# kit-cel/vae-equalizer

Hardware: AMD Instinct MI355X
Metric: equalized symbols/s/GPU, DP 64-QAM VAE-LE (higher is better)
Workload: dtype f32

## Files before the change

### vae_equalizer_amd/csrc/vaeq_dp_wave_kernel.h

```cpp
#pragma once
#include <hip/hip_runtime.h>
#include <stdint.h>
#include <type_traits>

#include "vaeq.h"
#include "vaeq_common.h"
#include "vaeq_launch.h"
#include "vaeq_wave.h"

#ifdef VAEQ_PHASE_STAMPS
#define VAEQ_STAMP(i) do { if (s == a.steps - 1) tst[i] = __builtin_readcyclecounter(); } while (0)
#define VAEQ_XSTAMP(i) do { if (s == a.steps - 1) tsx[i] = __builtin_readcyclecounter(); } while (0)
#else
#define VAEQ_STAMP(i) do { } while (0)
#define VAEQ_XSTAMP(i) do { } while (0)
#endif
#define VAEQ_NSTAMP 12
#ifndef VAEQ_PIPE
#define VAEQ_PIPE 1
#endif
#define VAEQ_BT_FRAMES 16
#ifndef VAEQ_WPS
#define VAEQ_WPS 2
#endif

namespace vaeq {

__device__ __forceinline__ float half_sum(float a0, float a1)
{
    const auto r = __builtin_amdgcn_permlane32_swap(__builtin_bit_cast(unsigned, a0), __builtin_bit_cast(unsigned, a1), false, false);
    return __builtin_bit_cast(float, (unsigned)r[0]) + __builtin_bit_cast(float, (unsigned)r[1]);
}

struct WaveLayout {
    int Lph, Uph;
    int X, E, U, PSv, W, H, PSh, VS, MOM, RED, XG, total;
};

__host__ __device__ inline WaveLayout wave_layout(int B, int M, int NW = 1)
{
    WaveLayout l;
    const int len = 2 * B + M - 1;
    const int lph = wave_lph(len);
    l.Lph = lph;
    l.Uph = B / 2 + 1;
    int o = 0;
    auto take = [&](int bytes) { int r = o; o += (bytes + 15) & ~15; return r; };
    l.X = take(2 * 4 * lph * 8);
    l.E = take(2 * 4 * lph * 8);
    const int ubytes = 2 * 2 * l.Uph * 8, gbytes = 2 * B * 8;
    l.U = take(ubytes > gbytes ? ubytes : gbytes);
    l.PSv = take(2 * (B + 1) * 4);
    l.W = take(2 * M * 16);
    l.H = take(2 * 2 * (M + 1) * 8);
    l.PSh = take(2 * (M + 1) * 4);
    l.VS = take(2 * M * 4);
    l.MOM = take(16 * 64 * 4);
    l.RED = take(NW > 1 ? 64 * 4 : 0);
    l.XG = take((NW - 1) * 4 * 64 * 4);
    l.total = o;
    return l;
}

struct CellCarry {
    static constexpr int fir_off(int g, int j, int Lph) { return g + (j < 4 ? j * Lph : (j - 4) * Lph + 1); }
    static constexpr int poly4(int c, int Lph) { return (c & 3) * Lph + (c >> 2); }
    static constexpr int d3_off(int b, int d, int mh, int Uph) { return (d & 1 ? Uph : 0) + (mh >> 1) - b + (d == -1 ? -1 : d == 2 ? 1 : 0); }
    static constexpr int poly2(int c, int Uph) { return (c & 1) * Uph + (c >> 1); }
    static constexpr bool fir_exact(int B, int M)
    {
        const int G = M / 4, len = 2 * B + M - 1, Lph = wave_lph(len);
        if (M % 4 != 1 || G < 2 || G % 2) return false;
        for (int g = 0; g < G; g++)
            for (int j = 0; j < 6; j++) {
                if (fir_off(g, j, Lph) != poly4(4 * g + j, Lph)) return false;
                if (4 * (B / 2 - 1) + 4 * g + j >= len) return false;
                if (g + 1 < G && j >= 4 && fir_off(g, j, Lph) != fir_off(g + 1, j - 4, Lph)) return false;
            }
        return poly4(4 * G, Lph) == fir_off(G - 1, 4, Lph) && 4 * (B / 2 - 1) + 4 * G + 2 < len;
    }
    static constexpr bool d3_exact(int B, int M)
    {
        const int mh = M / 2, NB = (mh + 1) / 2, Uph = B / 2 + 1, T = B - mh;
        if ((mh & 1) || NB < 2 || NB % 2) return false;
// ... 359 lines not shown
    char *sm = reinterpret_cast<char *>(smem4);
    const int gl = threadIdx.x, lane = NW > 1 ? (gl & 63) : gl, wv = NW > 1 ? (gl >> 6) : 0, run = blockIdx.x;
    constexpr int NT = 64 * NW, NP = 2 * NW;
    constexpr bool UNI = BT > 0 && uniform_parts(BT, M, NP);
    constexpr bool FIXL = BT > 0 || (BL > 0 && M != 13 && M != 17 && !(M == 31 && NW == 1));
    constexpr bool PIPE = VAEQ_PIPE && FIXL;
    constexpr bool WIDE = FIXL;
    constexpr bool B100 = BT == 100 && NW == 1;
    constexpr bool CARRY = B100 && M == 25 && PIPE && WIDE;
    constexpr int QAUX = B100 ? 2 : 0;
    const int B = BT ? BT : a.B;
    const int BS = BT ? BT : BL ? BL : B;
    constexpr bool ODDB = BT == 0 && BL > 0;
    const int L = 2 * B, nm = L - Mh, P2 = ODDB ? (B + 1) / 2 : B / 2;
    const float rnm = 1.0f / (float)nm;
    const WaveLayout lay = wave_layout(BS, M, NW);
    const int Lph = lay.Lph, Uph = lay.Uph;
    float2 *Xs = reinterpret_cast<float2 *>(sm + lay.X), *Es = reinterpret_cast<float2 *>(sm + lay.E);
    float2 *Us = reinterpret_cast<float2 *>(sm + lay.U), *GY = Us;
    float4 *Wt = reinterpret_cast<float4 *>(sm + lay.W);
    float2 *Ht = reinterpret_cast<float2 *>(sm + lay.H);
    float *PSv = reinterpret_cast<float *>(sm + lay.PSv);
    float *PSh = reinterpret_cast<float *>(sm + lay.PSh);
    float *VS = reinterpret_cast<float *>(sm + lay.VS);
    float *RED = reinterpret_cast<float *>(sm + lay.RED), *XG = reinterpret_cast<float *>(sm + lay.XG);

    float amp[NLEV], b2[NLEV], nlogP[NLEV];
    const float nusc = a.nu_sc[run];
#pragma unroll
    for (int i = 0; i < NLEV; i++) {
        amp[i] = a.amp[i];
        b2[i] = nusc * amp[i] * amp[i] * LOG2E;
        nlogP[i] = -logf(a.P[(size_t)run * NLEV + i]);
    }
    const float var0 = a.var[run * 2 + 0], var1 = a.var[run * 2 + 1];
    const float lrW = a.lr_W[run], lrH = a.lr_h[run];

    for (int i = gl; i < (lay.W - lay.X) / 8; i += NT) Xs[i] = make_float2(0.f, 0.f);
    for (int i = gl; i < (lay.PSh - lay.H) / 8; i += NT) Ht[i] = make_float2(0.f, 0.f);
    __syncthreads();
    const int tk = lane & 31, half = lane >> 5;
    const bool worker = tk < M, owner = worker && wv == 0;
    const int part = wv * 2 + half;
    const size_t gbase = (size_t)run * 8 * M;
    constexpr bool TP = BT == 100 && NW == 1 && M == 25;
    int oc = half, tj = tk;
    bool ownr = owner;
    if constexpr (TP) {
        oc = TapPairMap::c(lane, M);
        tj = TapPairMap::kept(lane, M);
        ownr = TapPairMap::owns(lane, M);
    }
    float *MOM = reinterpret_cast<float *>(sm + lay.MOM) + lane;
#define mWr(p) MOM[(0 + (p)) * 64]
#define mWi(p) MOM[(2 + (p)) * 64]
#define vWr(p) MOM[(4 + (p)) * 64]
#define vWi(p) MOM[(6 + (p)) * 64]
#define mHr(p) MOM[(8 + (p)) * 64]
#define mHi(p) MOM[(10 + (p)) * 64]
#define vHr(p) MOM[(12 + (p)) * 64]
#define vHi(p) MOM[(14 + (p)) * 64]
    if (ownr) {
#pragma unroll
        for (int p = 0; p < 2; p++) {
            const size_t ir = gbase + (oc * 4 + p) * M + tj, ii = gbase + (oc * 4 + 2 + p) * M + tj;
            float *wq = reinterpret_cast<float *>(&Wt[p * M + tj]);
            wq[oc * 2 + 0] = a.W[ir];
            wq[oc * 2 + 1] = a.W[ii];
            mWr(p) = a.adam_mW[ir]; mWi(p) = a.adam_mW[ii];
            vWr(p) = a.adam_vW[ir]; vWi(p) = a.adam_vW[ii];
            const size_t hr = gbase + ((oc * 2 + p) * 2 + 0) * M + tj, hi = hr + M;
            Ht[(oc * 2 + p) * MP + tj] = make_float2(a.h[hr], a.h[hi]);
            mHr(p) = a.adam_mh[hr]; mHi(p) = a.adam_mh[hi];
            vHr(p) = a.adam_vh[hr]; vHi(p) = a.adam_vh[hi];
        }
    }
    int step = a.step[run];
    __shared__ double BTW[2][VAEQ_BT_FRAMES];
    if (gl < VAEQ_BT_FRAMES && gl < a.n_frames) {
        const double t = (double)(step + gl * a.steps);
        BTW[0][gl] = pow(0.9, t);
        BTW[1][gl] = pow(0.999, t);
    }
    __syncthreads();
    double b1t = BTW[0][0], b2t = BTW[1][0];

    const int klen = a.keep_len, k0 = a.keep_off;
    const size_t No = (size_t)a.steps * klen;
    constexpr bool pairst = PAIR;
    const bool act = gl < P2;
    const int nq = (nm + 3) / 4;
    const int n0 = 2 * gl;
    const bool v1 = ODDB ? act && (n0 + 1 < B) : act;
    const float2 *Xl = Xs + gl, *El = Es + gl, *Ul = Us + gl;
    const float2 *Xa = Xs + (act ? gl : 0), *Ea = Es + (act ? gl : 0);

    const bool ldl = gl < (ODDB ? (L + 3) / 4 : L / 4);
    float4 pf[4];
    const uint32_t S4 = (uint32_t)a.S * 4u;
    auto frame_rsrc = [&](int f) { return make_rsrc(a.rx + ((size_t)run * a.n_frames + f) * 4 * (size_t)a.S, 4u * S4); };
    auto fetch = [&](const __amdgpu_buffer_rsrc_t xr, int s) {
        const uint32_t vo = ldl ? ((uint32_t)s * (uint32_t)a.stride_sym * 2u + 4u * gl) * 4u : OOB;
#pragma unroll
        for (int r = 0; r < 4; r++) pf[r] = bld128(xr, vo, (uint32_t)r * S4);
    };
#ifdef VAEQ_PHASE_STAMPS
    long long tst[VAEQ_NSTAMP], tsx[8];
#endif
    fetch(frame_rsrc(0), 0);
    for (int f = 0; f < a.n_frames; f++) {
        const __amdgpu_buffer_rsrc_t xr = frame_rsrc(f), xn = frame_rsrc(f + 1 < a.n_frames ? f + 1 : f);
        if (f && f < VAEQ_BT_FRAMES) {
            b1t = BTW[0][f];
            b2t = BTW[1][f];
// ... 111 lines not shown
                    }
                    if (df) {
                        float v0 = q[0].x, v1 = q[0].y;
                        int b0 = 0, b1 = 0;
#pragma unroll
                        for (int i = 1; i < NLEV; i++) {
                            if (q[i].x > v0) { v0 = q[i].x; b0 = i; }
                            if (q[i].y > v1) { v1 = q[i].y; b1 = i; }
                        }
                        const uint32_t ro = (uint32_t)(o * 2 + c) * (uint32_t)No;
                        if (pairst) bst16((unsigned short)(b0 | (b1 << 8)), dr, kept0 ? col : OOB, ro);
                        else { bst8((unsigned char)b0, dr, kept0 ? col : OOB, ro); bst8((unsigned char)b1, dr, kept1 ? col + 1u : OOB, ro); }
                    }
                    v2f m2 = {0.f, 0.f}, m3 = {0.f, 0.f}, kk = {0.f, 0.f}, kl = {0.f, 0.f};
#pragma unroll
                    for (int i = 0; i < NLEV; i++) {
                        const v2f d = amp[i] - m1, qd = q[i] * d, g = z[i] * LN2 + nlogP[i];
                        m2 += qd * d;
                        m3 += qd * d * d;
                        kk += qd * g;
                        kl += q[i] * g;
                    }
                    const bool inr0 = (n0 >= mh) && (n0 < B - mh) && act;
                    const bool inr1 = (n0 + 1 >= mh) && (n0 + 1 < B - mh) && act;
                    if (inr0) klsum += kl.x - __builtin_amdgcn_logf(ssum.x) * LN2;
                    if (inr1) klsum += kl.y - __builtin_amdgcn_logf(ssum.y) * LN2;
                    asm volatile("" : "+v"(m2), "+v"(m3), "+v"(kk), "+v"(klsum));
                    mv[0][o][c] = m2.x; mv[1][o][c] = m2.y;
                    mt3[0][o][c] = m3.x; mt3[1][o][c] = m3.y;
                    mkc[0][o][c] = inr0 ? kk.x : 0.f;
                    mkc[1][o][c] = inr1 ? kk.y : 0.f;
                    if (c) { muv[0].y = m1.x; muv[1].y = m1.y; } else { muv[0].x = m1.x; muv[1].x = m1.y; }
                    if (qf) {
#pragma unroll
                        for (int i = 0; i < NLEV; i++) {
                            const uint32_t ro = qrow;
                            if (pairst) bst64<QAUX>(q[i], qr, vo0, ro);
                            else { bst32<QAUX>(q[i].x, qr, vo0, ro); bst32<QAUX>(q[i].y, qr, vo1, ro); }
                            qrow += No4;
                            asm volatile("" : "+s"(qrow));
                        }
                    }
                }
                vv[o][0] = act ? mv[0][o][0] + mv[0][o][1] : 0.f;
                vv[o][1] = v1 ? mv[1][o][0] + mv[1][o][1] : 0.f;
                if (act) {
                    Us[(o * 2 + 0) * Uph + gl] = muv[0];
                    Us[(o * 2 + 1) * Uph + gl] = v1 ? muv[1] : make_float2(0.f, 0.f);
                }
            }
            VAEQ_STAMP(4);
            {
                float inc[2];
#pragma unroll
                for (int o = 0; o < 2; o++) inc[o] = wave_incl_scan_dpp(vv[o][0] + vv[o][1]);
                if constexpr (NW > 1) {
                    if (lane == 63) { RED[wv] = inc[0]; RED[NW + wv] = inc[1]; }
                    sync_lds<NW>();
#pragma unroll
                    for (int w = 0; w < NW - 1; w++)
                        if (w < wv) { inc[0] += RED[w]; inc[1] += RED[NW + w]; }
                }
#pragma unroll
                for (int o = 0; o < 2; o++) {
                    if (act) {
                        PSv[o * (BS + 1) + n0 + 1] = inc[o] - vv[o][1];
                        PSv[o * (BS + 1) + n0 + 2] = inc[o];
                    }
                    if (gl == 0) PSv[o * (BS + 1)] = 0.f;
                }
            }
            sync_lds<NW>();
            if (owner) {
                const int lo = (Mh - tk + 1) >> 1, hi_ = (nm - 1 + Mh - tk) >> 1;
                VS[half * M + tk] = PSv[half * (BS + 1) + hi_ + 1] - PSv[half * (BS + 1) + lo];
            }
            sync_lds<NW>();

            VAEQ_STAMP(5);
            float se0 = 0.f, se1 = 0.f;
            float hq0 = 0.f, hq1 = 0.f;
            if (worker) {
                const float2 h0 = Ht[(0 * 2 + half) * MP + tk], h1 = Ht[(1 * 2 + half) * MP + tk];
                hq0 = h0.x * h0.x + h0.y * h0.y;
                hq1 = h1.x * h1.x + h1.y * h1.y;
            }
            const float vsl = worker ? VS[half * M + tk] : 0.f;
            if constexpr (B100 && M == 25) {
                constexpr int T = 100 - mh, NB = (mh + 1) / 2;
                static_assert((mh & 1) == 0 && (Mh & 3) == 0 && D3Map::exact(100, M), "D3Map: mh even (a = mh stands alone, its odd tap is the pad)");
                const int l3 = lane;
                const int m3 = D3Map::m(l3, T), modd = m3 & 1, m3h = (3 * m3) >> 1;
                cacc D3[3][2];
                const int xo = D3Map::chi(l3) * 4 * Lph + (Mh >> 2) + m3h;
                const int o0 = xo + (modd ? 2 * Lph : 0), o2 = xo + (modd ? 1 : 2 * Lph);
                const int off[6] = {o0, o0 + Lph, o2, o2 + Lph, o0 + 1, o0 + Lph + 1};
                v2f x6[6];
#pragma unroll
                for (int k = 0; k < 6; k++) x6[k] = lds2(Xs + off[k]);
                {
                    const float2 *uE = Us + modd * Uph + m3h, *uO = Us + (modd ^ 1) * Uph + m3h + modd;
                    const float2 *hc = Ht + D3Map::chi(l3) * 2 * MP;
                    v2f am[2][4];
#pragma unroll
                    for (int v = 0; v < 2; v++) {
                        am[v][0] = lds2(hc + v * MP + Mh);
                        am[v][1] = lds2(uE + v * 2 * Uph); am[v][2] = lds2(uO + v * 2 * Uph); am[v][3] = lds2(uE + v * 2 * Uph + 1);
                    }
// ... 93 lines not shown
                    const float2 *h0 = Ht + (0 * 2 + v) * MP, *h1 = Ht + (1 * 2 + v) * MP;
                    const float2 *up = Us + (gl < nq ? gl : 0) + v * 2 * Uph;
                    auto step_a = [&](int aa, v2f ulo, v2f uhi, auto first) {
                        constexpr bool F = decltype(first)::value;
                        const v2f e0 = lds2(h0 + 2 * aa), o0 = lds2(h0 + 2 * aa + 1), e1 = lds2(h1 + 2 * aa), o1 = lds2(h1 + 2 * aa + 1);
                        cmacf<F>(D[0][0], e0, ulo); cmacf<F>(D[0][1], o0, ulo);
                        cmacf<F>(D[0][2], e0, uhi); cmacf<F>(D[0][3], o0, uhi);
                        cmacf<F>(D[1][0], e1, ulo); cmacf<F>(D[1][1], o1, ulo);
                        cmacf<F>(D[1][2], e1, uhi); cmacf<F>(D[1][3], o1, uhi);
                    };
                    if (NA & 1) {
                        if (v == 0) step_a(mh, lds2(up), lds2(up + Uph), std::true_type{});
                        else step_a(mh, lds2(up), lds2(up + Uph), std::false_type{});
                    } else if (v == 0) {
#pragma unroll
                        for (int chi = 0; chi < 2; chi++)
#pragma unroll
                            for (int i = 0; i < 4; i++) D[chi][i] = cacc0();
                    }
                    constexpr int ph = mh & 1;
                    auto load = [&](int b, v2f (&r)[11]) {
                        const int sl = (mh >> 1) - b;
                        r[0] = lds2(up + ph * Uph + sl);
                        r[1] = lds2(up + (ph ^ 1) * Uph + sl + ph);
                        r[2] = lds2(up + (ph ^ 1) * Uph + sl + ph - 1);
#pragma unroll
                        for (int t = 0; t < 4; t++) { r[3 + t] = lds2(h0 + 4 * b + t); r[7 + t] = lds2(h1 + 4 * b + t); }
                    };
                    auto fma = [&](int, const v2f (&r)[11], auto) {
                        cmac(D[0][0], r[3], r[0]); cmac(D[0][1], r[4], r[0]); cmac(D[0][2], r[3], r[1]); cmac(D[0][3], r[4], r[1]);
                        cmac(D[1][0], r[7], r[0]); cmac(D[1][1], r[8], r[0]); cmac(D[1][2], r[7], r[1]); cmac(D[1][3], r[8], r[1]);
                        cmac(D[0][0], r[5], r[2]); cmac(D[0][1], r[6], r[2]); cmac(D[0][2], r[5], r[0]); cmac(D[0][3], r[6], r[0]);
                        cmac(D[1][0], r[9], r[2]); cmac(D[1][1], r[10], r[2]); cmac(D[1][2], r[9], r[0]); cmac(D[1][3], r[10], r[0]);
                    };
                    pipe2<11, false, PIPE>(NB, load, fma);
                }
                VAEQ_STAMP(6);
                if (gl < nq) {
#pragma unroll
                    for (int chi = 0; chi < 2; chi++)
#pragma unroll
                        for (int i = 0; i < 4; i++) {
                            const int ce = Mh + i;
                            const float2 x = Xl[(chi * 4 + (ce & 3)) * Lph + (ce >> 2)];
                            const float2 Dv = cfin(D[chi][i]);
                            float2 e = make_float2(x.x - Dv.x, x.y - Dv.y);
                            if (4 * gl + i >= nm) e = make_float2(0.f, 0.f);
                            Es[(chi * 4 + (ce & 3)) * Lph + gl + (ce >> 2)] = e;
                            const float e2 = e.x * e.x + e.y * e.y;
                            if (chi) se1 += e2; else se0 += e2;
                        }
                }
            }
            se0 = wave_sum_dpp(se0);
            se1 = wave_sum_dpp(se1);
            klsum = wave_sum_dpp(klsum);
            if constexpr (NW > 1) {
                if (lane == 0) { RED[16 + wv] = se0; RED[16 + NW + wv] = se1; RED[16 + 2 * NW + wv] = klsum; }
                sync_lds<NW>();
                se0 = RED[16]; se1 = RED[16 + NW]; klsum = RED[16 + 2 * NW];
#pragma unroll
                for (int w = 1; w < NW; w++) { se0 += RED[16 + w]; se1 += RED[16 + NW + w]; klsum += RED[16 + 2 * NW + w]; }
            }
            const float C0 = se0 + wave_sum_dpp(hq0 * vsl), C1 = se1 + wave_sum_dpp(hq1 * vsl);
            const float gC0 = (float)nm * __builtin_amdgcn_rcpf(C0), gC1 = (float)nm * __builtin_amdgcn_rcpf(C1);
            {
                const uint32_t vo = gl == 0 ? 0u : OOB;
                if (a.loss) bst32((float)nm * LN2 * (__builtin_amdgcn_logf(C0) + __builtin_amdgcn_logf(C1)) + klsum, lr_, vo, (uint32_t)s * 4u);
                if (a.var_est) {
                    bst32(C0 * rnm, vr_, vo, (uint32_t)s * 4u);
                    bst32(C1 * rnm, vr_, vo, ((uint32_t)a.steps + (uint32_t)s) * 4u);
                }
            }
            {
                const float inc = half_incl_scan_dpp(gC0 * hq0 + gC1 * hq1);
                if (owner) PSh[half * MP + tk + 1] = inc;
                if (tk == 0) PSh[half * MP] = 0.f;
            }
            sync_lds<NW>();

            VAEQ_STAMP(7);
            step += 1;
            b1t *= 0.9;
            b2t *= 0.999;
            const float rbc1 = __builtin_amdgcn_rcpf((float)(1.0 - b1t));
            const float bc2s = __builtin_amdgcn_rcpf(__builtin_amdgcn_sqrtf((float)(1.0 - b2t)));
            const float ssW = lrW * rbc1, ssH = lrH * rbc1;
            float2 hnew[2];
            hnew[0] = hnew[1] = make_float2(0.f, 0.f);
            float ghr[2] = {0, 0}, ghi[2] = {0, 0};
            float2 hacc[2];
            {
                float2 ph_h[2] = {make_float2(0.f, 0.f), make_float2(0.f, 0.f)};
                float ph_vs[2] = {0.f, 0.f};
                if (NW == 1 && ownr) {
#pragma unroll
                    for (int v = 0; v < 2; v++) {
                        ph_h[v] = Ht[(oc * 2 + v) * MP + tj];
                        ph_vs[v] = VS[v * M + tj];
                    }
                }
                cacc ca[2][2];
                if constexpr (TP) {
                    static_assert(TapPairMap::exact(100, M) && UNI, "TapPairMap");
                    const int lt = lane;
                    constexpr int NH = TapPairMap::dh_pairs(100, M);
                    const int par = TapPairMap::par(lt, M), sl = TapPairMap::alo(lt, M) >> 1, ma = TapPairMap::part_h(lt, M) * NH;
                    const int ceA = par + Mh, ceB = par + Mh + 2;
                    const float2 *ec = Es + TapPairMap::c(lt, M) * 4 * Lph + ma;
                    const float2 *uA = Us + (mh >> 1) - sl + ma, *uB = uA + Uph;
                    const float2 *uC = TapPairMap::tap(lt, M, 1) < M ? uB - 1 : uA;
                    VAEQ_XSTAMP(0);
                    tap_pair_sum<NH, 1>(ca, ec + (ceA & 3) * Lph + (ceA >> 2), ec + (ceB & 3) * Lph + (ceB >> 2), uA, uB, 2 * Uph, uC);
                } else {
                    const int tkc = worker ? tk : 0, par = tkc & 1, aa = tkc >> 1;
                    const int T = (nm - par + 1) >> 1, Th = ((T + 2 * NP - 1) / (2 * NP)) << 1;
                    const int ma = (part * Th) >> 1, mb = (min(T, part * Th + Th) + 1) >> 1;
                    const int ceA = par + Mh, ceB = par + Mh + 2, npA = mh - aa, npB = mh - aa + 1;
                    const float2 *eA = Es + (ceA & 3) * Lph + (ceA >> 2) + ma, *eB = Es + (ceB & 3) * Lph + (ceB >> 2) + ma;
                    const float2 *uA = Us + (npA & 1) * Uph + (npA >> 1) + ma, *uB = Us + (npB & 1) * Uph + (npB >> 1) + ma;
                    auto load1 = [&](int m, v2f *r) {
                        r[0] = lds2(eA + m); r[1] = lds2(eA + 4 * Lph + m); r[2] = lds2(uA + m); r[3] = lds2(uA + 2 * Uph + m);
                        r[4] = lds2(eB + m); r[5] = lds2(eB + 4 * Lph + m); r[6] = lds2(uB + m); r[7] = lds2(uB + 2 * Uph + m);
                    };
                    cacc cbx[2][2];
                    cacc (&cb)[2][2] = WIDE ? cbx : ca;
                    auto fma1 = [&](const v2f *r, auto first) {
                        constexpr bool F = decltype(first)::value;
                        cmacf<F>(ca[0][0], r[2], r[0]); cmacf<F>(ca[0][1], r[3], r[0]); cmacf<F>(ca[1][0], r[2], r[1]); cmacf<F>(ca[1][1], r[3], r[1]);
                        cmacf<F && WIDE>(cb[0][0], r[6], r[4]); cmacf<F && WIDE>(cb[0][1], r[7], r[4]); cmacf<F && WIDE>(cb[1][0], r[6], r[5]); cmacf<F && WIDE>(cb[1][1], r[7], r[5]);
                    };
                    auto load = [&](int i, v2f (&r)[16]) { load1(2 * i, r); load1(2 * i + 1, r + 8); };
                    auto fma = [&](int, const v2f (&r)[16], auto first) { fma1(r, first); fma1(r + 8, std::false_type{}); };
                    int n = mb - ma;
                    VAEQ_XSTAMP(0);
                    if constexpr (UNI) {
                        n = __builtin_amdgcn_readfirstlane(n);
                        pipe2<16, true, PIPE>(n >> 1, load, fma);
                    } else {
                        ca[0][0] = ca[0][1] = ca[1][0] = ca[1][1] = cbx[0][0] = cbx[0][1] = cbx[1][0] = cbx[1][1] = cacc0();
                        pipe2<16, false, PIPE>(n >> 1, load, fma);
                    }
                    if (n & 1) {
                        v2f r[8];
                        load1(n - 1, r);
                        fma1(r, std::false_type{});
                    }
                    if constexpr (WIDE) {
#pragma unroll
                        for (int i = 0; i < 2; i++)
#pragma unroll
                            for (int j = 0; j < 2; j++) { ca[i][j].a += cbx[i][j].a; ca[i][j].b += cbx[i][j].b; }
                    }
                }
                VAEQ_XSTAMP(1);
                float2 acc[2][2];
#pragma unroll
                for (int chi = 0; chi < 2; chi++)
#pragma unroll
                    for (int v = 0; v < 2; v++) acc[chi][v] = cfinc(ca[chi][v]);
                if constexpr (B100) {
#pragma unroll
                    for (int v = 0; v < 2; v++) {
                        acc[0][v].x = acc[1][v].x = half_sum(acc[0][v].x, acc[1][v].x);
                        acc[0][v].y = acc[1][v].y = half_sum(acc[0][v].y, acc[1][v].y);
                    }
                } else {
#pragma unroll
                    for (int chi = 0; chi < 2; chi++)
#pragma unroll
                        for (int v = 0; v < 2; v++) {
                            acc[chi][v].x += __shfl_xor(acc[chi][v].x, 32, 64);
                            acc[chi][v].y += __shfl_xor(acc[chi][v].y, 32, 64);
                        }
                }
                if constexpr (NW > 1) {
#pragma unroll
                    for (int v = 0; v < 2; v++) {
                        hacc[v] = half ? acc[1][v] : acc[0][v];
                        if (wv > 0) {
                            XG[((wv - 1) * 4 + 2 * v + 0) * 64 + lane] = hacc[v].x;
                            XG[((wv - 1) * 4 + 2 * v + 1) * 64 + lane] = hacc[v].y;
                        }
                    }
                }
                VAEQ_XSTAMP(2);
                if (NW == 1 && ownr) {
                    const float g = oc ? gC1 : gC0;
#pragma unroll
                    for (int v = 0; v < 2; v++) {
                        const float2 ac = half ? acc[1][v] : acc[0][v];
                        const float2 hh = ph_h[v];
                        const float vs = ph_vs[v];
                        ghr[v] = g * (-2.0f * ac.x + 2.0f * hh.x * vs);
                        ghi[v] = g * (-2.0f * ac.y + 2.0f * hh.y * vs);
                        hnew[v] = hh;
                        if (!a.no_update) {
                            adam_update_fast(hnew[v].x, mHr(v), vHr(v), ghr[v], ssH, bc2s);
                            adam_update_fast(hnew[v].y, mHi(v), vHi(v), ghi[v], ssH, bc2s);
                        }
                    }
                }
            }

            asm volatile("" : "+v"(hnew[0].x), "+v"(hnew[0].y), "+v"(hnew[1].x), "+v"(hnew[1].y), "+v"(ghr[0]), "+v"(ghr[1]), "+v"(ghi[0]),
                         "+v"(ghi[1]));
            {
                const bool last_s = s + 1 == a.steps;
                if constexpr (B100) {
                    const bool more = !(last_s && f + 1 == a.n_frames);
                    const uint32_t vo = ldl && more ? ((uint32_t)(last_s ? 0 : s + 1) * (uint32_t)a.stride_sym * 2u + 4u * gl) * 4u : OOB;
#pragma unroll
                    for (int r = 0; r < 4; r++) pf[r] = bld128(last_s ? xn : xr, vo, (uint32_t)r * S4);
                } else if (!(last_s && f + 1 == a.n_frames)) fetch(last_s ? xn : xr, last_s ? 0 : s + 1);
            }
            VAEQ_XSTAMP(3);
            VAEQ_STAMP(8);
            float2 gy[2][2];
            {
                float2 au0[2][2], au1[2][2];
                {
                    cacc cu[2][2][2];
                    pair_du<M, WIDE, CARRY>(cu, Ea, Lph, Ht, MP);
#pragma unroll
                    for (int sy = 0; sy < 2; sy++)
#pragma unroll
                        for (int v = 0; v < 2; v++) { au0[sy][v] = cfinc(cu[0][sy][v]); au1[sy][v] = cfinc(cu[1][sy][v]); }
                }
#pragma unroll
                for (int sy = 0; sy < 2; sy++) {
                    const int sx = 2 * (n0 + sy);
                    const int jlo = max(0, Mh - sx), jhi = max(jlo - 1, min(Mh, nm - 1 + Mh - sx));
#pragma unroll
                    for (int v = 0; v < 2; v++) {
                        const float ur = -2.0f * (gC0 * au0[sy][v].x + gC1 * au1[sy][v].x);
                        const float ui = -2.0f * (gC0 * au0[sy][v].y + gC1 * au1[sy][v].y);
                        const float gv = PSh[v * MP + jhi + 1] - PSh[v * MP + jlo];
                        const float iv = 1.0f / (v ? var1 : var0);
                        gy[sy][v].x = iv * (ur * mv[sy][v][0] + gv * mt3[sy][v][0] + mkc[sy][v][0]);
                        gy[sy][v].y = iv * (ui * mv[sy][v][1] + gv * mt3[sy][v][1] + mkc[sy][v][1]);
                    }
                }
            }
            VAEQ_STAMP(9);
            sync_lds<NW>();
            if constexpr (NW > 1) {
                if (owner) {
                    const float g = half ? gC1 : gC0;
#pragma unroll
                    for (int v = 0; v < 2; v++) {
                        float2 ac = hacc[v];
#pragma unroll
                        for (int w = 0; w < NW - 1; w++) {
                            ac.x += XG[(w * 4 + 2 * v + 0) * 64 + lane];
                            ac.y += XG[(w * 4 + 2 * v + 1) * 64 + lane];
                        }
                        const float2 hh = Ht[(half * 2 + v) * MP + tk];
                        const float vs = VS[v * M + tk];
                        ghr[v] = g * (-2.0f * ac.x + 2.0f * hh.x * vs);
                        ghi[v] = g * (-2.0f * ac.y + 2.0f * hh.y * vs);
                        hnew[v] = hh;
                        if (!a.no_update) {
                            adam_update_fast(hnew[v].x, mHr(v), vHr(v), ghr[v], ssH, bc2s);
                            adam_update_fast(hnew[v].y, mHi(v), vHi(v), ghi[v], ssH, bc2s);
                        }
                    }
                }
            }
            if (act) {
#pragma unroll
                for (int v = 0; v < 2; v++) {
                    GY[v * BS + n0] = gy[0][v];
                    GY[v * BS + n0 + 1] = v1 ? gy[1][v] : make_float2(0.f, 0.f);
                }
            }
            if (ownr && !a.no_update) {
                Ht[(oc * 2 + 0) * MP + tj] = hnew[0];
                Ht[(oc * 2 + 1) * MP + tj] = hnew[1];
            }
            sync_lds<NW>();

            VAEQ_STAMP(10);
            float gwr[2] = {0, 0}, gwi[2] = {0, 0};
            {
                float pw_w[2][2] = {{0.f, 0.f}, {0.f, 0.f}}, pw_m[2][2] = {{0.f, 0.f}, {0.f, 0.f}}, pw_v[2][2] = {{0.f, 0.f}, {0.f, 0.f}};
                if (ownr) {
#pragma unroll
                    for (int p = 0; p < 2; p++) {
                        const float *wq = reinterpret_cast<const float *>(&Wt[p * M + tj]) + oc * 2;
                        pw_w[p][0] = wq[0]; pw_w[p][1] = wq[1];
                        pw_m[p][0] = mWr(p); pw_m[p][1] = mWi(p);
                        pw_v[p][0] = vWr(p); pw_v[p][1] = vWi(p);
                    }
                }
                cacc ca[2][2];
                if constexpr (TP) {
                    const int lt = lane;
                    constexpr int NQ = TapPairMap::dw_pairs(100);
                    const int cA = TapPairMap::tap(lt, M, 1), cB = cA + 2, ma = TapPairMap::part_w(lt) * NQ;
                    const float2 *gA = GY + TapPairMap::c(lt, M) * BS + 2 * ma;
                    const float2 *xA = Xs + (cA & 3) * Lph + (cA >> 2) + ma, *xB = Xs + (cB & 3) * Lph + (cB >> 2) + ma;
                    cacc cr[2][2];
                    VAEQ_XSTAMP(4);
                    tap_pair_sum<NQ, 2>(cr, gA, gA + 1, xA, xB, 4 * Lph, xB - 1);
#pragma unroll
                    for (int p = 0; p < 2; p++) { ca[0][p] = cr[1][p]; ca[1][p] = cr[0][p]; }
                } else {
                    const int tkc = worker ? tk : 0;
                    const int Be = ODDB ? B + (B & 1) : B;
                    const int Bq = ((Be + 2 * NP - 1) / (2 * NP)) << 1;
                    const int ma = (part * Bq) >> 1, mb = min(Be, part * Bq + Bq) >> 1;
                    const int cA = tkc, cB = tkc + 2;
                    const float2 *xA = Xs + (cA & 3) * Lph + (cA >> 2) + ma, *xB = Xs + (cB & 3) * Lph + (cB >> 2) + ma;
                    const float2 *G0 = GY + 2 * ma, *G1 = GY + BS + 2 * ma;
                    auto load1 = [&](int m, v2f *r) {
                        r[0] = lds2(G0 + 2 * m); r[1] = lds2(G0 + 2 * m + 1); r[2] = lds2(G1 + 2 * m); r[3] = lds2(G1 + 2 * m + 1);
                        r[4] = lds2(xA + m); r[5] = lds2(xA + 4 * Lph + m); r[6] = lds2(xB + m); r[7] = lds2(xB + 4 * Lph + m);
                    };
                    cacc cbx[2][2];
                    cacc (&cb)[2][2] = WIDE ? cbx : ca;
                    auto fma1 = [&](const v2f *r, auto first) {
                        constexpr bool F = decltype(first)::value;
                        cmacf<F>(ca[0][0], r[4], r[0]); cmacf<F>(ca[0][1], r[5], r[0]); cmacf<F>(ca[1][0], r[4], r[2]); cmacf<F>(ca[1][1], r[5], r[2]);
                        cmacf<F && WIDE>(cb[0][0], r[6], r[1]); cmacf<F && WIDE>(cb[0][1], r[7], r[1]); cmacf<F && WIDE>(cb[1][0], r[6], r[3]); cmacf<F && WIDE>(cb[1][1], r[7], r[3]);
                    };
                    auto load = [&](int i, v2f (&r)[16]) { load1(2 * i, r); load1(2 * i + 1, r + 8); };
                    auto fma = [&](int, const v2f (&r)[16], auto first) { fma1(r, first); fma1(r + 8, std::false_type{}); };
                    int n = mb - ma;
                    VAEQ_XSTAMP(4);
                    if constexpr (UNI) {
                        n = __builtin_amdgcn_readfirstlane(n);
                        pipe2<16, true, PIPE>(n >> 1, load, fma);
                    } else {
                        ca[0][0] = ca[0][1] = ca[1][0] = ca[1][1] = cbx[0][0] = cbx[0][1] = cbx[1][0] = cbx[1][1] = cacc0();
                        pipe2<16, false, PIPE>(n >> 1, load, fma);
                    }
                    if (n & 1) {
                        v2f r[8];
                        load1(n - 1, r);
                        fma1(r, std::false_type{});
                    }
                    if constexpr (WIDE) {
#pragma unroll
                        for (int i = 0; i < 2; i++)
#pragma unroll
                            for (int j = 0; j < 2; j++) { ca[i][j].a += cbx[i][j].a; ca[i][j].b += cbx[i][j].b; }
                    }
                }
                VAEQ_XSTAMP(5);
                float2 acc[2][2];
#pragma unroll
                for (int o = 0; o < 2; o++)
#pragma unroll
                    for (int pp = 0; pp < 2; pp++) acc[o][pp] = cfinc(ca[o][pp]);
                if constexpr (B100) {
#pragma unroll
                    for (int p = 0; p < 2; p++) {
                        acc[0][p].x = acc[1][p].x = half_sum(acc[0][p].x, acc[1][p].x);
                        acc[0][p].y = acc[1][p].y = half_sum(acc[0][p].y, acc[1][p].y);
                    }
                } else {
#pragma unroll
                    for (int o = 0; o < 2; o++)
#pragma unroll
                        for (int p = 0; p < 2; p++) {
                            acc[o][p].x += __shfl_xor(acc[o][p].x, 32, 64);
                            acc[o][p].y += __shfl_xor(acc[o][p].y, 32, 64);
                        }
                }
                if constexpr (NW > 1) {
#pragma unroll
                    for (int p = 0; p < 2; p++) {
                        const float2 ac = half ? acc[1][p] : acc[0][p];
                        if (wv > 0) {
                            XG[((wv - 1) * 4 + 2 * p + 0) * 64 + lane] = ac.x;
                            XG[((wv - 1) * 4 + 2 * p + 1) * 64 + lane] = ac.y;
                        }
                    }
                    sync_lds<NW>();
                }
                VAEQ_XSTAMP(6);
                if (ownr) {
#pragma unroll
                    for (int p = 0; p < 2; p++) {
                        float2 ac = half ? acc[1][p] : acc[0][p];
                        if constexpr (NW > 1) {
#pragma unroll
                            for (int w = 0; w < NW - 1; w++) {
                                ac.x += XG[(w * 4 + 2 * p + 0) * 64 + lane];
                                ac.y += XG[(w * 4 + 2 * p + 1) * 64 + lane];
                            }
                        }
                        gwr[p] = ac.x;
                        gwi[p] = ac.y;
                        if (!a.no_update) {
                            float *wq = reinterpret_cast<float *>(&Wt[p * M + tj]) + oc * 2;
                            float wr = pw_w[p][0], wi = pw_w[p][1];
                            adam_update_fast(wr, pw_m[p][0], pw_v[p][0], gwr[p], ssW, bc2s);
                            adam_update_fast(wi, pw_m[p][1], pw_v[p][1], gwi[p], ssW, bc2s);
                            wq[0] = wr;
                            wq[1] = wi;
                            mWr(p) = pw_m[p][0]; mWi(p) = pw_m[p][1];
                            vWr(p) = pw_v[p][0]; vWi(p) = pw_v[p][1];
                        }
                    }
                }
            }
            if (a.dbg_gW && ownr && f == a.n_frames - 1 && s == a.steps - 1) {
#pragma unroll
                for (int p = 0; p < 2; p++) {
                    a.dbg_gW[gbase + (oc * 4 + p) * M + tj] = gwr[p];
                    a.dbg_gW[gbase + (oc * 4 + 2 + p) * M + tj] = gwi[p];
                    a.dbg_gh[gbase + ((oc * 2 + p) * 2 + 0) * M + tj] = ghr[p];
                    a.dbg_gh[gbase + ((oc * 2 + p) * 2 + 1) * M + tj] = ghi[p];
                }
            }
            sync_lds<NW>();
            VAEQ_XSTAMP(7);
            VAEQ_STAMP(11);
        }
    }
#ifdef VAEQ_PHASE_STAMPS
    if (gl == 0 && run == (int)gridDim.x / 2 && a.loss)
        for (int i = 0; i + 1 < VAEQ_NSTAMP; i++) a.loss[i] = (float)(tst[i + 1] - tst[i]);
    if (gl == 0 && run == (int)gridDim.x / 2 && a.loss)
        for (int i = 0; i < 7; i++) a.loss[16 + i] = (float)(tsx[i + 1] - tsx[i]);
#endif

    if (ownr && !a.no_update) {
#pragma unroll
        for (int p = 0; p < 2; p++) {
            const size_t ir = gbase + (oc * 4 + p) * M + tj, ii = gbase + (oc * 4 + 2 + p) * M + tj;
            const float *wq = reinterpret_cast<const float *>(&Wt[p * M + tj]) + oc * 2;
            a.W[ir] = wq[0]; a.W[ii] = wq[1];
            a.adam_mW[ir] = mWr(p); a.adam_mW[ii] = mWi(p);
            a.adam_vW[ir] = vWr(p); a.adam_vW[ii] = vWi(p);
            const size_t hr = gbase + ((oc * 2 + p) * 2 + 0) * M + tj, hi = hr + M;
            const float2 hh = Ht[(oc * 2 + p) * MP + tj];
            a.h[hr] = hh.x; a.h[hi] = hh.y;
            a.adam_mh[hr] = mHr(p); a.adam_mh[hi] = mHi(p);
            a.adam_vh[hr] = vHr(p); a.adam_vh[hi] = vHi(p);
        }
    }
    if (gl == 0 && !a.no_update) a.step[run] = step;
#undef mWr
#undef mWi
#undef vWr
#undef vWi
#undef mHr
#undef mHi
#undef vHr
#undef vHi
}


template <int M, int NLEV, int BT, int NW, int BL, bool SPEC>
static int launch_wave(const vaeq_dp_args &a, hipStream_t st)
{
    const size_t lds = (size_t)wave_layout(BL ? BL : a.B, M, NW).total;
    const bool pair = ((a.keep_len | a.keep_off) & 1) == 0;
    const int out = !SPEC ? 0 : (!a.eq_out && !a.dec_out) ? 1 : !a.q_out ? 2 : 0;
    constexpr int O1 = SPEC ? 1 : 0, O2 = SPEC ? 2 : 0;
    void (*const k[2][3])(const vaeq_dp_args) = {
        {dp_wave_kernel<M, NLEV, BT, false, 0, NW, BL>, dp_wave_kernel<M, NLEV, BT, false, O1, NW, BL>, dp_wave_kernel<M, NLEV, BT, false, O2, NW, BL>},
        {dp_wave_kernel<M, NLEV, BT, true, 0, NW, BL>, dp_wave_kernel<M, NLEV, BT, true, O1, NW, BL>, dp_wave_kernel<M, NLEV, BT, true, O2, NW, BL>}};
    note_kernel("vaeq::dp_wave_kernel<%d, %d, %d, %s, %d, %d, %d>", M, NLEV, BT, pair ? "true" : "false", out, NW, BL);
    return launch(k[pair][out], dim3(a.R), dim3(64 * NW), lds, st, a);
}

template <int M, int NLEV, int BT, int NW, int BL>
static int64_t wave_resident(int B)
{
    int nb = 0, dev = 0;
    hipDeviceProp_t prop;
    if (hipGetDevice(&dev) != hipSuccess || hipGetDeviceProperties(&prop, dev) != hipSuccess) return VAEQ_ERR_DEVICE;
    auto k = dp_wave_kernel<M, NLEV, BT, true, 0, NW, BL>;
    if (hipOccupancyMaxActiveBlocksPerMultiprocessor(&nb, k, 64 * NW, (size_t)wave_layout(BL ? BL : B, M, NW).total) != hipSuccess) return VAEQ_ERR_DEVICE;
    return (int64_t)nb * prop.multiProcessorCount;
}

template <int M, int BT, int NW>
static int launch_wave_lev(const vaeq_dp_args &a, hipStream_t st)
{
    return dispatch_nlev(a.n_lev, [&](auto nl) { return launch_wave<M, decltype(nl)::value, BT, NW, 0, (BT > 0)>(a, st); });
}
template <int M, int BT, int NW>
static int64_t wave_resident_lev(int B, int n_lev)
{
    return dispatch_nlev(n_lev, [&](auto nl) { return wave_resident<M, decltype(nl)::value, BT, NW, 0>(B); });
}
template <int M, int BL, int NW, bool SPEC>
static int launch_wave_fixl_lev(const vaeq_dp_args &a, hipStream_t st)
{
    return dispatch_nlev(a.n_lev, [&](auto nl) { return launch_wave<M, decltype(nl)::value, 0, NW, BL, SPEC>(a, st); });
}
template <int M, int BL, int NW>
static int64_t wave_resident_fixl_lev(int n_lev)
// ... 34 lines not shown
```

### vae_equalizer_amd/csrc/vaeq_wave.h

```cpp
#pragma once
#include <hip/hip_runtime.h>
#include <stdint.h>
#include <type_traits>

namespace vaeq {

__device__ __forceinline__ void wave_lds_sync() { asm volatile("" ::: "memory"); }

template <int NW>
__device__ __forceinline__ void sync_lds()
{
    if constexpr (NW == 1) wave_lds_sync();
    else asm volatile("s_waitcnt lgkmcnt(0)\n\ts_barrier" ::: "memory");
}

template <int NW, int K>
__device__ __forceinline__ void waves_sum(float (&v)[K], float *red, int lane, int wv)
{
    if constexpr (NW > 1) {
        if (lane == 0) {
#pragma unroll
            for (int k = 0; k < K; k++) red[k * NW + wv] = v[k];
        }
        sync_lds<NW>();
// ... 150 lines not shown

__device__ __forceinline__ v2f cfin2(const cacc &c)
{
    v2f r;
    asm("v_pk_add_f32 %0, %1, %2 op_sel:[0,1] op_sel_hi:[1,0] neg_lo:[0,1]" : "=v"(r) : "v"(c.a), "v"(c.b));
    return r;
}
__device__ __forceinline__ v2f cfinc2(const cacc &c)
{
    v2f r;
    asm("v_pk_add_f32 %0, %1, %2 op_sel:[0,1] op_sel_hi:[1,0] neg_hi:[0,1]" : "=v"(r) : "v"(c.a), "v"(c.b));
    return r;
}
__device__ __forceinline__ float2 cfin(const cacc &c) { const v2f r = cfin2(c); return make_float2(r.x, r.y); }
__device__ __forceinline__ float2 cfinc(const cacc &c) { const v2f r = cfinc2(c); return make_float2(r.x, r.y); }

template <int CTRL, int ROW_MASK = 0xF, int BANK_MASK = 0xF>
__device__ __forceinline__ float dpp_f(float v)
{
    return __builtin_bit_cast(float, __builtin_amdgcn_update_dpp(0, __builtin_bit_cast(int, v), CTRL, ROW_MASK, BANK_MASK, true));
}
__device__ __forceinline__ float wave_sum_dpp(float v)
{
    v += dpp_f<0xB1>(v);
    v += dpp_f<0x4E>(v);
    v += dpp_f<0x141>(v);
    v += dpp_f<0x140>(v);
    v += dpp_f<0x142, 0xA>(v);
    v += dpp_f<0x143, 0xC>(v);
    return __builtin_bit_cast(float, __builtin_amdgcn_readlane(__builtin_bit_cast(int, v), 63));
}
__device__ __forceinline__ float row_incl_scan_dpp(float v)
{
    float s = v + dpp_f<0x111>(v);
    s += dpp_f<0x112>(v);
    s += dpp_f<0x113>(v);
    s += dpp_f<0x114, 0xF, 0xE>(s);
    s += dpp_f<0x118, 0xF, 0xC>(s);
    return s;
}
__device__ __forceinline__ float half_incl_scan_dpp(float v)
{
    float s = row_incl_scan_dpp(v);
    s += dpp_f<0x142, 0xA>(s);
    return s;
}
__device__ __forceinline__ float wave_incl_scan_dpp(float v)
{
    float s = half_incl_scan_dpp(v);
    s += dpp_f<0x143, 0xC>(s);
    return s;
}

__device__ __forceinline__ float wave_incl_scan(float v, int lane)
{
#pragma unroll
    for (int d = 1; d < 64; d <<= 1) {
        const float t = __shfl_up(v, d, 64);
        if (lane >= d) v += t;
    }
    return v;
}

__host__ __device__ constexpr inline int wave_lph(int len)
{
    int lph = (len + 3) / 4 + 1;
    while ((lph & 31) != 8 && (lph & 31) != 24) lph++;
    return lph;
}

}
```

Before: 11.30 billion.

## Batch DPP reductions/scans and packed Adam updates on all lanes for B=100 path

For the B=100 tap-pair path, five wave sums are fused into one interleaved inline-asm DPP sequence and two inclusive scans are interleaved. The per-component half_sum calls become one packed half_sum2, and the h and W Adam updates use packed v2f math. These updates now run on every lane, with only owner lanes writing back, which removes the owner-lane branches. The Adam moment layout in LDS is reordered so real and imaginary parts sit next to each other. Together this is meant to cut instruction latency and divergence on the serial per-step critical path. The cost is hand-written DPP asm with manual s_nop hazard handling, and non-owner lanes reading LDS cells they do not own.

```diff
diff --git a/vae_equalizer_amd/csrc/vaeq_dp_wave_kernel.h b/vae_equalizer_amd/csrc/vaeq_dp_wave_kernel.h
--- a/vae_equalizer_amd/csrc/vaeq_dp_wave_kernel.h
+++ b/vae_equalizer_amd/csrc/vaeq_dp_wave_kernel.h
@@ -26,10 +26,25 @@
 
 namespace vaeq {
 
-__device__ __forceinline__ float half_sum(float a0, float a1)
-{
-    const auto r = __builtin_amdgcn_permlane32_swap(__builtin_bit_cast(unsigned, a0), __builtin_bit_cast(unsigned, a1), false, false);
-    return __builtin_bit_cast(float, (unsigned)r[0]) + __builtin_bit_cast(float, (unsigned)r[1]);
+__device__ __forceinline__ v2f half_sum2(v2f a0, v2f a1)
+{
+    const float a0x = a0.x, a0y = a0.y, a1x = a1.x, a1y = a1.y;
+    const auto rx = __builtin_amdgcn_permlane32_swap(__builtin_bit_cast(unsigned, a0x), __builtin_bit_cast(unsigned, a1x), false, false);
+    const auto ry = __builtin_amdgcn_permlane32_swap(__builtin_bit_cast(unsigned, a0y), __builtin_bit_cast(unsigned, a1y), false, false);
+    v2f r0 = {__builtin_bit_cast(float, (unsigned)rx[0]), __builtin_bit_cast(float, (unsigned)ry[0])};
+    v2f r1 = {__builtin_bit_cast(float, (unsigned)rx[1]), __builtin_bit_cast(float, (unsigned)ry[1])};
+    asm volatile("" : "+v"(r0), "+v"(r1));
+    return r0 + r1;
+}
+
+__device__ __forceinline__ void adam_update_fast2(v2f &p, v2f &m, v2f &v, v2f g, float step_size, float rbc2s)
+{
+    m = __builtin_elementwise_fma(g - m, v2f{0.1f, 0.1f}, m);
+    v = v * 0.999f;
+    v = __builtin_elementwise_fma(0.001f * g, g, v);
+    const float d0 = fmaf(__builtin_amdgcn_sqrtf(v.x), rbc2s, 1e-8f), d1 = fmaf(__builtin_amdgcn_sqrtf(v.y), rbc2s, 1e-8f);
+    const v2f rd = {__builtin_amdgcn_rcpf(d0), __builtin_amdgcn_rcpf(d1)};
+    p = __builtin_elementwise_fma(-step_size * m, rd, p);
 }
 
 struct WaveLayout {
@@ -495,14 +510,15 @@
         ownr = TapPairMap::owns(lane, M);
     }
     float *MOM = reinterpret_cast<float *>(sm + lay.MOM) + lane;
-#define mWr(p) MOM[(0 + (p)) * 64]
-#define mWi(p) MOM[(2 + (p)) * 64]
-#define vWr(p) MOM[(4 + (p)) * 64]
-#define vWi(p) MOM[(6 + (p)) * 64]
-#define mHr(p) MOM[(8 + (p)) * 64]
-#define mHi(p) MOM[(10 + (p)) * 64]
-#define vHr(p) MOM[(12 + (p)) * 64]
-#define vHi(p) MOM[(14 + (p)) * 64]
+#define VAEQ_MOM(base, im, p) MOM[((base) + (BT == 100 && NW == 1 ? 2 * (p) + (im) : 2 * (im) + (p))) * 64]
+#define mWr(p) VAEQ_MOM(0, 0, p)
+#define mWi(p) VAEQ_MOM(0, 1, p)
+#define vWr(p) VAEQ_MOM(4, 0, p)
+#define vWi(p) VAEQ_MOM(4, 1, p)
+#define mHr(p) VAEQ_MOM(8, 0, p)
+#define mHi(p) VAEQ_MOM(8, 1, p)
+#define vHr(p) VAEQ_MOM(12, 0, p)
+#define vHi(p) VAEQ_MOM(12, 1, p)
     if (ownr) {
 #pragma unroll
         for (int p = 0; p < 2; p++) {
@@ -720,8 +736,14 @@
             VAEQ_STAMP(4);
             {
                 float inc[2];
-#pragma unroll
-                for (int o = 0; o < 2; o++) inc[o] = wave_incl_scan_dpp(vv[o][0] + vv[o][1]);
+                if constexpr (B100) {
+                    inc[0] = vv[0][0] + vv[0][1];
+                    inc[1] = vv[1][0] + vv[1][1];
+                    wave_incl_scan2_dpp_keep(inc[0], inc[1]);
+                } else {
+#pragma unroll
+                    for (int o = 0; o < 2; o++) inc[o] = wave_incl_scan_dpp(vv[o][0] + vv[o][1]);
+                }
                 if constexpr (NW > 1) {
                     if (lane == 63) { RED[wv] = inc[0]; RED[NW + wv] = inc[1]; }
                     sync_lds<NW>();
@@ -921,9 +943,16 @@
                         }
                 }
             }
-            se0 = wave_sum_dpp(se0);
-            se1 = wave_sum_dpp(se1);
-            klsum = wave_sum_dpp(klsum);
+            float hv0 = 0.f, hv1 = 0.f;
+            if constexpr (B100) {
+                float ws[5] = {wave_sum_first(se0), wave_sum_first(se1), wave_sum_first(klsum), wave_sum_first(hq0, vsl), wave_sum_first(hq1, vsl)};
+                wave_sum5_dpp_keep(ws);
+                se0 = ws[0]; se1 = ws[1]; klsum = ws[2]; hv0 = ws[3]; hv1 = ws[4];
+            } else {
+                se0 = wave_sum_dpp(se0);
+                se1 = wave_sum_dpp(se1);
+                klsum = wave_sum_dpp(klsum);
+            }
             if constexpr (NW > 1) {
                 if (lane == 0) { RED[16 + wv] = se0; RED[16 + NW + wv] = se1; RED[16 + 2 * NW + wv] = klsum; }
                 sync_lds<NW>();
@@ -931,7 +960,14 @@
 #pragma unroll
                 for (int w = 1; w < NW; w++) { se0 += RED[16 + w]; se1 += RED[16 + NW + w]; klsum += RED[16 + 2 * NW + w]; }
             }
-            const float C0 = se0 + wave_sum_dpp(hq0 * vsl), C1 = se1 + wave_sum_dpp(hq1 * vsl);
+            float C0, C1;
+            if constexpr (B100) {
+                C0 = se0 + hv0;
+                C1 = se1 + hv1;
+            } else {
+                C0 = se0 + wave_sum_dpp(hq0 * vsl);
+                C1 = se1 + wave_sum_dpp(hq1 * vsl);
+            }
             const float gC0 = (float)nm * __builtin_amdgcn_rcpf(C0), gC1 = (float)nm * __builtin_amdgcn_rcpf(C1);
             {
                 const uint32_t vo = gl == 0 ? 0u : OOB;
@@ -962,7 +998,8 @@
             {
                 float2 ph_h[2] = {make_float2(0.f, 0.f), make_float2(0.f, 0.f)};
                 float ph_vs[2] = {0.f, 0.f};
-                if (NW == 1 && ownr) {
+                static_assert(!B100 || TP, "B = 100: every lane updates -- the cells a lane without a tap names are inside the LDS allocation for TapPairMap (M = 25) only");
+                if (B100 || (NW == 1 && ownr)) {
 #pragma unroll
                     for (int v = 0; v < 2; v++) {
                         ph_h[v] = Ht[(oc * 2 + v) * MP + tj];
@@ -1023,18 +1060,34 @@
                     }
                 }
                 VAEQ_XSTAMP(1);
-                float2 acc[2][2];
-#pragma unroll
-                for (int chi = 0; chi < 2; chi++)
-#pragma unroll
-                    for (int v = 0; v < 2; v++) acc[chi][v] = cfinc(ca[chi][v]);
                 if constexpr (B100) {
+                    v2f sum[2];
+#pragma unroll
+                    for (int v = 0; v < 2; v++) sum[v] = half_sum2(cfinc2(ca[0][v]), cfinc2(ca[1][v]));
+                    VAEQ_XSTAMP(2);
+                    const float g = oc ? gC1 : gC0;
 #pragma unroll
                     for (int v = 0; v < 2; v++) {
-                        acc[0][v].x = acc[1][v].x = half_sum(acc[0][v].x, acc[1][v].x);
-                        acc[0][v].y = acc[1][v].y = half_sum(acc[0][v].y, acc[1][v].y);
+                        v2f hh = {ph_h[v].x, ph_h[v].y};
+                        const v2f gh = g * __builtin_elementwise_fma(2.0f * hh, v2f{ph_vs[v], ph_vs[v]}, -2.0f * sum[v]);
+                        if (!a.no_update) {
+                            v2f mo = {mHr(v), mHi(v)}, vo = {vHr(v), vHi(v)};
+                            adam_update_fast2(hh, mo, vo, gh, ssH, bc2s);
+                            mHr(v) = mo.x; mHi(v) = mo.y;
+                            vHr(v) = vo.x; vHi(v) = vo.y;
+                        }
+                        hnew[v] = f2(hh);
+                        if (a.dbg_gW && ownr && f == a.n_frames - 1 && s == a.steps - 1) {
+                            a.dbg_gh[gbase + ((oc * 2 + v) * 2 + 0) * M + tj] = gh.x;
+                            a.dbg_gh[gbase + ((oc * 2 + v) * 2 + 1) * M + tj] = gh.y;
+                        }
                     }
                 } else {
+                    float2 acc[2][2];
+#pragma unroll
+                    for (int chi = 0; chi < 2; chi++)
+#pragma unroll
+                        for (int v = 0; v < 2; v++) acc[chi][v] = cfinc(ca[chi][v]);
 #pragma unroll
                     for (int chi = 0; chi < 2; chi++)
 #pragma unroll
@@ -1042,38 +1095,39 @@
                             acc[chi][v].x += __shfl_xor(acc[chi][v].x, 32, 64);
                             acc[chi][v].y += __shfl_xor(acc[chi][v].y, 32, 64);
                         }
-                }
-                if constexpr (NW > 1) {
-#pragma unroll
-                    for (int v = 0; v < 2; v++) {
-                        hacc[v] = half ? acc[1][v] : acc[0][v];
-                        if (wv > 0) {
-                            XG[((wv - 1) * 4 + 2 * v + 0) * 64 + lane] = hacc[v].x;
-                            XG[((wv - 1) * 4 + 2 * v + 1) * 64 + lane] = hacc[v].y;
-                        }
-                    }
-                }
-                VAEQ_XSTAMP(2);
-                if (NW == 1 && ownr) {
-                    const float g = oc ? gC1 : gC0;
-#pragma unroll
-                    for (int v = 0; v < 2; v++) {
-                        const float2 ac = half ? acc[1][v] : acc[0][v];
-                        const float2 hh = ph_h[v];
-                        const float vs = ph_vs[v];
-                        ghr[v] = g * (-2.0f * ac.x + 2.0f * hh.x * vs);
-                        ghi[v] = g * (-2.0f * ac.y + 2.0f * hh.y * vs);
-                        hnew[v] = hh;
-                        if (!a.no_update) {
-                            adam_update_fast(hnew[v].x, mHr(v), vHr(v), ghr[v], ssH, bc2s);
-                            adam_update_fast(hnew[v].y, mHi(v), vHi(v), ghi[v], ssH, bc2s);
-                        }
-                    }
-                }
-            }
-
-            asm volatile("" : "+v"(hnew[0].x), "+v"(hnew[0].y), "+v"(hnew[1].x), "+v"(hnew[1].y), "+v"(ghr[0]), "+v"(ghr[1]), "+v"(ghi[0]),
-                         "+v"(ghi[1]));
+                    if constexpr (NW > 1) {
+#pragma unroll
+                        for (int v = 0; v < 2; v++) {
+                            hacc[v] = half ? acc[1][v] : acc[0][v];
+                            if (wv > 0) {
+                                XG[((wv - 1) * 4 + 2 * v + 0) * 64 + lane] = hacc[v].x;
+                                XG[((wv - 1) * 4 + 2 * v + 1) * 64 + lane] = hacc[v].y;
+                            }
+                        }
+                    }
+                    VAEQ_XSTAMP(2);
+                    if (NW == 1 && ownr) {
+                        const float g = oc ? gC1 : gC0;
+#pragma unroll
+                        for (int v = 0; v < 2; v++) {
+                            const float2 ac = half ? acc[1][v] : acc[0][v];
+                            const float2 hh = ph_h[v];
+                            const float vs = ph_vs[v];
+                            ghr[v] = g * (-2.0f * ac.x + 2.0f * hh.x * vs);
+                            ghi[v] = g * (-2.0f * ac.y + 2.0f * hh.y * vs);
+                            hnew[v] = hh;
+                            if (!a.no_update) {
+                                adam_update_fast(hnew[v].x, mHr(v), vHr(v), ghr[v], ssH, bc2s);
+                                adam_update_fast(hnew[v].y, mHi(v), vHi(v), ghi[v], ssH, bc2s);
+                            }
+                        }
+                    }
+                }
+            }
+
+            if constexpr (B100) asm volatile("" : "+v"(hnew[0].x), "+v"(hnew[0].y), "+v"(hnew[1].x), "+v"(hnew[1].y));
+            else asm volatile("" : "+v"(hnew[0].x), "+v"(hnew[0].y), "+v"(hnew[1].x), "+v"(hnew[1].y), "+v"(ghr[0]), "+v"(ghr[1]), "+v"(ghi[0]),
+                              "+v"(ghi[1]));
             {
                 const bool last_s = s + 1 == a.steps;
                 if constexpr (B100) {
@@ -1153,7 +1207,7 @@
             float gwr[2] = {0, 0}, gwi[2] = {0, 0};
             {
                 float pw_w[2][2] = {{0.f, 0.f}, {0.f, 0.f}}, pw_m[2][2] = {{0.f, 0.f}, {0.f, 0.f}}, pw_v[2][2] = {{0.f, 0.f}, {0.f, 0.f}};
-                if (ownr) {
+                if (B100 || ownr) {
 #pragma unroll
                     for (int p = 0; p < 2; p++) {
                         const float *wq = reinterpret_cast<const float *>(&Wt[p * M + tj]) + oc * 2;
@@ -1217,18 +1271,33 @@
                     }
                 }
                 VAEQ_XSTAMP(5);
-                float2 acc[2][2];
-#pragma unroll
-                for (int o = 0; o < 2; o++)
-#pragma unroll
-                    for (int pp = 0; pp < 2; pp++) acc[o][pp] = cfinc(ca[o][pp]);
                 if constexpr (B100) {
+                    v2f sum[2];
+#pragma unroll
+                    for (int p = 0; p < 2; p++) sum[p] = half_sum2(cfinc2(ca[0][p]), cfinc2(ca[1][p]));
+                    VAEQ_XSTAMP(6);
 #pragma unroll
                     for (int p = 0; p < 2; p++) {
-                        acc[0][p].x = acc[1][p].x = half_sum(acc[0][p].x, acc[1][p].x);
-                        acc[0][p].y = acc[1][p].y = half_sum(acc[0][p].y, acc[1][p].y);
+                        gwr[p] = sum[p].x;
+                        gwi[p] = sum[p].y;
+                        if (!a.no_update) {
+                            v2f w = {pw_w[p][0], pw_w[p][1]}, mo = {pw_m[p][0], pw_m[p][1]}, vo = {pw_v[p][0], pw_v[p][1]};
+                            adam_update_fast2(w, mo, vo, sum[p], ssW, bc2s);
+                            if (ownr) {
+                                float *wq = reinterpret_cast<float *>(&Wt[p * M + tj]) + oc * 2;
+                                wq[0] = w.x;
+                                wq[1] = w.y;
+                                mWr(p) = mo.x; mWi(p) = mo.y;
+                                vWr(p) = vo.x; vWi(p) = vo.y;
+                            }
+                        }
                     }
                 } else {
+                    float2 acc[2][2];
+#pragma unroll
+                    for (int o = 0; o < 2; o++)
+#pragma unroll
+                        for (int pp = 0; pp < 2; pp++) acc[o][pp] = cfinc(ca[o][pp]);
 #pragma unroll
                     for (int o = 0; o < 2; o++)
 #pragma unroll
@@ -1236,41 +1305,41 @@
                             acc[o][p].x += __shfl_xor(acc[o][p].x, 32, 64);
                             acc[o][p].y += __shfl_xor(acc[o][p].y, 32, 64);
                         }
-                }
-                if constexpr (NW > 1) {
-#pragma unroll
-                    for (int p = 0; p < 2; p++) {
-                        const float2 ac = half ? acc[1][p] : acc[0][p];
-                        if (wv > 0) {
-                            XG[((wv - 1) * 4 + 2 * p + 0) * 64 + lane] = ac.x;
-                            XG[((wv - 1) * 4 + 2 * p + 1) * 64 + lane] = ac.y;
-                        }
-                    }
-                    sync_lds<NW>();
-                }
-                VAEQ_XSTAMP(6);
-                if (ownr) {
-#pragma unroll
-                    for (int p = 0; p < 2; p++) {
-                        float2 ac = half ? acc[1][p] : acc[0][p];
-                        if constexpr (NW > 1) {
-#pragma unroll
-                            for (int w = 0; w < NW - 1; w++) {
-                                ac.x += XG[(w * 4 + 2 * p + 0) * 64 + lane];
-                                ac.y += XG[(w * 4 + 2 * p + 1) * 64 + lane];
+                    if constexpr (NW > 1) {
+#pragma unroll
+                        for (int p = 0; p < 2; p++) {
+                            const float2 ac = half ? acc[1][p] : acc[0][p];
+                            if (wv > 0) {
+                                XG[((wv - 1) * 4 + 2 * p + 0) * 64 + lane] = ac.x;
+                                XG[((wv - 1) * 4 + 2 * p + 1) * 64 + lane] = ac.y;
                             }
                         }
-                        gwr[p] = ac.x;
-                        gwi[p] = ac.y;
-                        if (!a.no_update) {
-                            float *wq = reinterpret_cast<float *>(&Wt[p * M + tj]) + oc * 2;
-                            float wr = pw_w[p][0], wi = pw_w[p][1];
-                            adam_update_fast(wr, pw_m[p][0], pw_v[p][0], gwr[p], ssW, bc2s);
-                            adam_update_fast(wi, pw_m[p][1], pw_v[p][1], gwi[p], ssW, bc2s);
-                            wq[0] = wr;
-                            wq[1] = wi;
-                            mWr(p) = pw_m[p][0]; mWi(p) = pw_m[p][1];
-                            vWr(p) = pw_v[p][0]; vWi(p) = pw_v[p][1];
+                        sync_lds<NW>();
+                    }
+                    VAEQ_XSTAMP(6);
+                    if (ownr) {
+#pragma unroll
+                        for (int p = 0; p < 2; p++) {
+                            float2 ac = half ? acc[1][p] : acc[0][p];
+                            if constexpr (NW > 1) {
+#pragma unroll
+                                for (int w = 0; w < NW - 1; w++) {
+                                    ac.x += XG[(w * 4 + 2 * p + 0) * 64 + lane];
+                                    ac.y += XG[(w * 4 + 2 * p + 1) * 64 + lane];
+                                }
+                            }
+                            gwr[p] = ac.x;
+                            gwi[p] = ac.y;
+                            if (!a.no_update) {
+                                float *wq = reinterpret_cast<float *>(&Wt[p * M + tj]) + oc * 2;
+                                float wr = pw_w[p][0], wi = pw_w[p][1];
+                                adam_update_fast(wr, pw_m[p][0], pw_v[p][0], gwr[p], ssW, bc2s);
+                                adam_update_fast(wi, pw_m[p][1], pw_v[p][1], gwi[p], ssW, bc2s);
+                                wq[0] = wr;
+                                wq[1] = wi;
+                                mWr(p) = pw_m[p][0]; mWi(p) = pw_m[p][1];
+                                vWr(p) = pw_v[p][0]; vWi(p) = pw_v[p][1];
+                            }
                         }
                     }
                 }
@@ -1280,8 +1349,10 @@
                 for (int p = 0; p < 2; p++) {
                     a.dbg_gW[gbase + (oc * 4 + p) * M + tj] = gwr[p];
                     a.dbg_gW[gbase + (oc * 4 + 2 + p) * M + tj] = gwi[p];
-                    a.dbg_gh[gbase + ((oc * 2 + p) * 2 + 0) * M + tj] = ghr[p];
-                    a.dbg_gh[gbase + ((oc * 2 + p) * 2 + 1) * M + tj] = ghi[p];
+                    if constexpr (!B100) {
+                        a.dbg_gh[gbase + ((oc * 2 + p) * 2 + 0) * M + tj] = ghr[p];
+                        a.dbg_gh[gbase + ((oc * 2 + p) * 2 + 1) * M + tj] = ghi[p];
+                    }
                 }
             }
             sync_lds<NW>();
@@ -1312,6 +1383,7 @@
         }
     }
     if (gl == 0 && !a.no_update) a.step[run] = step;
+#undef VAEQ_MOM
 #undef mWr
 #undef mWi
 #undef vWr
diff --git a/vae_equalizer_amd/csrc/vaeq_wave.h b/vae_equalizer_amd/csrc/vaeq_wave.h
--- a/vae_equalizer_amd/csrc/vaeq_wave.h
+++ b/vae_equalizer_amd/csrc/vaeq_wave.h
@@ -226,6 +226,43 @@
     return s;
 }
 
+#define VAEQ_DPPK(i, ctrl) "v_add_f32_dpp %" #i ", %" #i ", %" #i " " ctrl "\n\t"
+#define VAEQ_DPPK2(ctrl) VAEQ_DPPK(0, ctrl) VAEQ_DPPK(1, ctrl)
+#define VAEQ_DPPK5(ctrl) VAEQ_DPPK2(ctrl) VAEQ_DPPK(2, ctrl) VAEQ_DPPK(3, ctrl) VAEQ_DPPK(4, ctrl)
+#define VAEQ_DPP_FULL " row_mask:0xf bank_mask:0xf"
+__device__ __forceinline__ float wave_sum_first(float v) { return v + dpp_f<0xB1>(v); }
+__device__ __forceinline__ float wave_sum_first(float a, float b) { return __builtin_fmaf(a, b, dpp_f<0xB1>(a * b)); }
+__device__ __forceinline__ void wave_sum5_dpp_keep(float (&v)[5])
+{
+    asm("s_nop 4\n\t"
+        VAEQ_DPPK5("quad_perm:[2,3,0,1]" VAEQ_DPP_FULL)
+        VAEQ_DPPK5("row_half_mirror" VAEQ_DPP_FULL)
+        VAEQ_DPPK5("row_mirror" VAEQ_DPP_FULL)
+        VAEQ_DPPK5("row_bcast:15 row_mask:0xa bank_mask:0xf")
+        VAEQ_DPPK5("row_bcast:31 row_mask:0xc bank_mask:0xf")
+        : "+v"(v[0]), "+v"(v[1]), "+v"(v[2]), "+v"(v[3]), "+v"(v[4]));
+#pragma unroll
+    for (int k = 0; k < 5; k++) v[k] = __builtin_bit_cast(float, __builtin_amdgcn_readlane(__builtin_bit_cast(int, v[k]), 63));
+}
+__device__ __forceinline__ void wave_incl_scan2_dpp_keep(float &a, float &b)
+{
+    float s0 = a + dpp_f<0x111>(a), s1 = b + dpp_f<0x111>(b);
+    s0 += dpp_f<0x112>(a); s1 += dpp_f<0x112>(b);
+    s0 += dpp_f<0x113>(a); s1 += dpp_f<0x113>(b);
+    asm("s_nop 4\n\t"
+        VAEQ_DPPK2("row_shr:4 row_mask:0xf bank_mask:0xe") "s_nop 0\n\t"
+        VAEQ_DPPK2("row_shr:8 row_mask:0xf bank_mask:0xc") "s_nop 0\n\t"
+        VAEQ_DPPK2("row_bcast:15 row_mask:0xa bank_mask:0xf") "s_nop 0\n\t"
+        VAEQ_DPPK2("row_bcast:31 row_mask:0xc bank_mask:0xf")
+        : "+v"(s0), "+v"(s1));
+    a = s0;
+    b = s1;
+}
+#undef VAEQ_DPPK
+#undef VAEQ_DPPK2
+#undef VAEQ_DPPK5
+#undef VAEQ_DPP_FULL
+
 __device__ __forceinline__ float wave_incl_scan(float v, int lane)
 {
 #pragma unroll
```

Measured after the change: 11.46 billion (median of 6 runs). +1.4%, better.
